# Veason-silverbullet/NNR

Measured on AMD Instinct MI355X. Metric: training impressions/sec on MIND-200k (CNE+SUE, bs=64), higher is better.
Workload: dtype f32

## Files before the change

nnr_amd/csrc/gemm.hip:

```cpp
#include "common.h"
#include <stdlib.h>
#include <type_traits>

namespace {

template <int BK>
__device__ __forceinline__ int swz(int r16) {
  return BK == 16 ? ((4 - (r16 >> 2)) & 3) : BK == 32 ? ((r16 >> 1) & 7) : (r16 & 15);
}

template <int TM, int TN>
__device__ __forceinline__ void gemm_epilogue(const nnr_gemm_args& g, f32x4 (&acc)[TM][TN], float* lds, float* __restrict__ C, int m0,
                                              int n0, int M, int N, int z) {
  constexpr int BN = 16 * TN, E_LD = BN + 4;
  const int tid = threadIdx.x, lane = tid & 63, w = tid >> 6;
  const int r = lane & 15, kk = lane >> 4;
  const uint32_t dthr = g.drop_thresh;
  const float dscale = g.drop_scale;
  const bool use_atomic = !g.slab_mode && (g.atomic || g.split_k > 1 || g.k_chunk > 0);
  float* aux = g.aux_out;
  const float* res = g.resid;
  const float* mulp = g.mul;
  if (g.batch > 1 && g.split_k <= 1 && g.k_chunk <= 0) {
    if (aux) aux += (long)z * g.stride_aux;
// ... 783 lines not shown
  if (nv == TN) run(std::true_type{});
  else run(std::false_type{});
  __syncthreads();
  gemm_epilogue<TM, TN>(g, acc, lds, C, m0, n0, M, N, z);
}

constexpr int kNtRagged = 1;

template <int TM, int TN, int NS, int OCC>
int launch_pipe2(const nnr_gemm_args& g0, hipStream_t s) {
  constexpr int BM = 64 * TM, BN = 16 * TN;
  nnr_gemm_args g = g0;
  g.sched = kNtRagged;
  const int nbm = (g.M + BM - 1) / BM, nbn = (g.N + BN - 1) / BN;
  dim3 grid(nbm * nbn, 1, g.batch > 1 ? g.batch : 1), block(256);
  hipLaunchKernelGGL((gemm_nt_pipe2_kernel<TM, TN, NS, OCC>), grid, block, 0, s, g);
  NNR_CHECK_LAUNCH();
  return NNR_OK;
}

template <int TM, int TN, int BK, int NS, int OCC, int PRIO = 0>
int launch_pipe(const nnr_gemm_args& g0, hipStream_t s) {
  constexpr int BM = 64 * TM, BN = 16 * TN;
  nnr_gemm_args g = g0;
  g.sched = kNtRagged;
  const int nbm = (g.M + BM - 1) / BM, nbn = (g.N + BN - 1) / BN;
  dim3 grid(nbm * nbn, 1, g.batch > 1 ? g.batch : 1), block(256);
  hipLaunchKernelGGL((gemm_nt_pipe_kernel<TM, TN, BK, NS, OCC, PRIO>), grid, block, 0, s, g);
  NNR_CHECK_LAUNCH();
  return NNR_OK;
}

static bool pipe_ok(const nnr_gemm_args& g) {
  auto al = [](const void* p) { return ((uintptr_t)p & 15) == 0; };
  return !g.trans_a && !g.trans_b && !g.b_idx && g.split_k <= 1 && g.k_chunk <= 0 && !g.rowdot_w && !g.colsum_out &&
         (g.drop_target == 0 || g.drop_target == 3 || g.drop_target == 4) && (g.K & 3) == 0 && (g.lda & 3) == 0 && (g.ldb & 3) == 0 &&
         al(g.A) && al(g.B) && (g.batch <= 1 || (((g.strideA | g.strideB) & 3) == 0)) && (g.dyn_dim == 0 || g.dyn_dim == 1);
}

typedef __bf16 bf16x8_t __attribute__((ext_vector_type(8)));
__device__ __forceinline__ void split3_bf16(float x, __bf16& h1, __bf16& h2, __bf16& h3) {
  const unsigned u = __builtin_bit_cast(unsigned, x), mag = u & 0x7fffffffu;
  const bool big = mag >= 0x7f7f8000u, nonfinite = mag >= 0x7f800000u;
  h1 = (__bf16)x;
  if (big) h1 = __builtin_bit_cast(__bf16, (unsigned short)((u >> 16) | (mag > 0x7f800000u ? 0x40u : 0u)));
  const float r1 = nonfinite ? 0.f : x - (float)h1;
  h2 = (__bf16)r1;
  const float r2 = r1 - (float)h2;
  h3 = (__bf16)r2;
}
__global__ void split_bf16x3_kernel(const float* __restrict__ w, int rows, int cols, int ld, int ldo, __bf16* __restrict__ out, long img_stride) {
  const long total = (long)rows * ldo;
  for (long i = blockIdx.x * (long)blockDim.x + threadIdx.x; i < total; i += (long)gridDim.x * blockDim.x) {
    const int r = (int)(i / ldo), c = (int)(i - (long)r * ldo);
    __bf16 a, b, d;
    split3_bf16(c < cols ? w[(long)r * ld + c] : 0.f, a, b, d);
    out[i] = a; out[img_stride + i] = b; out[2 * img_stride + i] = d;
  }
}
__device__ __forceinline__ int bx3_swzA(int r) { return ((r >> 1) & 1) | (((r >> 3) & 1) << 2); }
__device__ __forceinline__ int bx3_swzB(int r) { return (r >> 1) & 3; }

typedef unsigned u32x4_t __attribute__((ext_vector_type(4)));
__device__ __forceinline__ unsigned hi16_pair(float odd, float even) {
  return __builtin_amdgcn_perm(__float_as_uint(odd), __float_as_uint(even), 0x07060302u);
}
__device__ __forceinline__ void split3_trunc8(const f32x4& x0, const f32x4& x1, bf16x8_t& a1, bf16x8_t& a2, bf16x8_t& a3) {
  const float xs[8] = {x0[0], x0[1], x0[2], x0[3], x1[0], x1[1], x1[2], x1[3]};
  unsigned w1[4], w2[4], w3[4];
#pragma unroll
  for (int p = 0; p < 4; ++p) {
    const float xe = xs[2 * p], xo = xs[2 * p + 1];
    const unsigned h1 = hi16_pair(xo, xe);
    const float re = xe - __uint_as_float(h1 << 16), ro = xo - __uint_as_float(h1 & 0xffff0000u);
    const unsigned h2 = hi16_pair(ro, re);
    const float se = re - __uint_as_float(h2 << 16), so = ro - __uint_as_float(h2 & 0xffff0000u);
    w1[p] = h1; w2[p] = h2; w3[p] = hi16_pair(so, se);
  }
  a1 = __builtin_bit_cast(bf16x8_t, u32x4_t{w1[0], w1[1], w1[2], w1[3]});
  a2 = __builtin_bit_cast(bf16x8_t, u32x4_t{w2[0], w2[1], w2[2], w2[3]});
  a3 = __builtin_bit_cast(bf16x8_t, u32x4_t{w3[0], w3[1], w3[2], w3[3]});
}

template <int TM, int TN, int NS>
__global__ __launch_bounds__(256, (NS * (64 * TM * 128 + 3 * 16 * TN * 64) > 80 * 1024 ? 1 : 2)) void gemm_nt_bx3_kernel(nnr_gemm_args g) {
  constexpr int BM = 64 * TM, BN = 16 * TN, BK = 32;
  constexpr int A_BYTES = BM * BK * 4, B_IMG_BYTES = BN * BK * 2, STAGE_BYTES = A_BYTES + 3 * B_IMG_BYTES;
  constexpr int NIA = A_BYTES / 1024, NIB1 = B_IMG_BYTES / 1024;
  static_assert(A_BYTES % 1024 == 0 && B_IMG_BYTES % 1024 == 0 && NIA % 4 == 0, "tile shape");
  constexpr int E_LD = BN + 4;
  constexpr int LDS_BYTES = NS * STAGE_BYTES > 64 * E_LD * 4 ? NS * STAGE_BYTES : 64 * E_LD * 4;
  __shared__ __attribute__((aligned(1024))) unsigned char lds_raw[LDS_BYTES];
  const int tid = threadIdx.x, lane = tid & 63, w = __builtin_amdgcn_readfirstlane(tid >> 6), r = lane & 15, q = lane >> 4;
  int M = g.M;
  if (g.dyn_dim == 1) M = min(M, *g.dyn_dev);
  const int N = g.N, K = g.K;
  const int nbm = (M + BM - 1) / BM, nbn = (N + BN - 1) / BN, nblk = nbm * nbn;
  if ((int)blockIdx.x >= nblk) return;
  int v;
  {
    const int b = blockIdx.x, qq = nblk >> 3, rem = nblk & 7, x = b & 7, slot = b >> 3;
    v = x * qq + min(x, rem) + slot;
  }
  const int bm = v / nbn, bn = v - bm * nbn, m0 = bm * BM, n0 = bn * BN;
  const int S = (K + BK - 1) / BK;
  const unsigned lds_base = (unsigned)(uintptr_t)lds_raw;
  const float* zero = nnr_zero_page;
  asm volatile("" : "+s"(zero));
  constexpr int NA = NIA / 4, NBW = (3 * NIB1 + 3) / 4;
  static_assert(NA <= 8 && NBW <= 8, "tile shape");
  unsigned voffA[8], voffB[8];
  int akc[NA], bkc[NBW];
#pragma unroll
  for (int i = 0; i < 8; ++i) voffA[i] = voffB[i] = 0;
#pragma unroll
  for (int i = 0; i < NA; ++i) {
    const int row = (w + 4 * i) * 8 + lane / 8, c = (lane % 8) ^ bx3_swzA(row & 15);
    akc[i] = 4 * c;
    voffA[i] = (unsigned)(((long)min(row, M - 1 - m0) * g.lda + 4 * c) * 4);
  }
#pragma unroll
  for (int j = 0; j < NBW; ++j) {
    const int idx = min(w + 4 * j, 3 * NIB1 - 1);
    const int img = idx / NIB1, jj = idx - img * NIB1, row = jj * 16 + lane / 4, c = (lane % 4) ^ bx3_swzB(row & 15);
    bkc[j] = 8 * c;
    voffB[j] = (unsigned)(((long)img * g.b3_stride + (long)min(row, N - 1 - n0) * g.ldb3 + 8 * c) * 2);
  }
  const float* Abase = g.A + (long)m0 * g.lda;
  const char* Bbase = reinterpret_cast<const char*>(reinterpret_cast<const __bf16*>(g.B3) + (long)n0 * g.ldb3);
  const bool nb_hi = ((3 * NIB1) % 4 == 0) || (w < (3 * NIB1) % 4);
  const bool ktail = (K % BK) != 0;
  auto issue = [&](int s) __attribute__((always_inline)) {
    const int k0 = s * BK;
    const unsigned sb = lds_base + (unsigned)((s % NS) * STAGE_BYTES) + (unsigned)(w * 1024);
    if (!(ktail && s == S - 1)) {
      lds_dma16_block<NA>(Abase + k0, sb, voffA);
      const float* bb = reinterpret_cast<const float*>(Bbase + 2L * k0);
      if (nb_hi) lds_dma16_block<NBW>(bb, sb + A_BYTES, voffB);
      else if constexpr (NBW > 1) lds_dma16_block<NBW - 1>(bb, sb + A_BYTES, voffB);
      return;
    }
#pragma unroll
    for (int i = 0; i < NA; ++i)
      lds_dma16((k0 + akc[i] < K) ? reinterpret_cast<const float*>(reinterpret_cast<const char*>(Abase + k0) + voffA[i]) : zero, sb + (unsigned)(i * 4096));
#pragma unroll
    for (int j = 0; j < NBW; ++j)
      if (j < NBW - 1 || nb_hi)
        lds_dma16((k0 + bkc[j] < K) ? reinterpret_cast<const float*>(Bbase + 2L * k0 + voffB[j]) : zero, sb + A_BYTES + (unsigned)(j * 4096));
  };
  f32x4 acc_hi[TM][TN], acc_lo[TM][TN];
#pragma unroll
  for (int m = 0; m < TM; ++m)
#pragma unroll
    for (int n = 0; n < TN; ++n) acc_hi[m][n] = acc_lo[m][n] = f32x4{0.f, 0.f, 0.f, 0.f};
#pragma unroll
  for (int s = 0; s < NS - 1; ++s)
    if (s < S) issue(s);
  for (int s = 0; s < S; ++s) {
    if (nb_hi) wait_stages<NA + NBW, NS - 2>(S - 1 - s);
    else wait_stages<NA + NBW - 1, NS - 2>(S - 1 - s);
    __builtin_amdgcn_s_barrier();
    if (s + NS - 1 < S) issue(s + NS - 1);
    const unsigned char* st = lds_raw + (s % NS) * STAGE_BYTES;
    const float* As = reinterpret_cast<const float*>(st);
    const __bf16* Bi = reinterpret_cast<const __bf16*>(st + A_BYTES);
    bf16x8_t bf[3][TN];
#pragma unroll
    for (int img = 0; img < 3; ++img)
#pragma unroll
      for (int n = 0; n < TN; ++n)
        bf[img][n] = *reinterpret_cast<const bf16x8_t*>(Bi + img * (BN * BK) + (n * 16 + r) * BK + ((q ^ bx3_swzB(r)) * 8));
#pragma unroll
    for (int m = 0; m < TM; ++m) {
      const float* arow = As + ((w * TM + m) * 16 + r) * BK;
      const f32x4 x0 = *reinterpret_cast<const f32x4*>(arow + 4 * ((2 * q) ^ bx3_swzA(r)));
      const f32x4 x1 = *reinterpret_cast<const f32x4*>(arow + 4 * ((2 * q + 1) ^ bx3_swzA(r)));
      bf16x8_t a1, a2, a3;
      split3_trunc8(x0, x1, a1, a2, a3);
#pragma unroll
      for (int n = 0; n < TN; ++n) {
        acc_hi[m][n] = __builtin_amdgcn_mfma_f32_16x16x32_bf16(a1, bf[0][n], acc_hi[m][n], 0, 0, 0);
        acc_lo[m][n] = __builtin_amdgcn_mfma_f32_16x16x32_bf16(a3, bf[0][n], acc_lo[m][n], 0, 0, 0);
        acc_lo[m][n] = __builtin_amdgcn_mfma_f32_16x16x32_bf16(a1, bf[2][n], acc_lo[m][n], 0, 0, 0);
        acc_lo[m][n] = __builtin_amdgcn_mfma_f32_16x16x32_bf16(a2, bf[1][n], acc_lo[m][n], 0, 0, 0);
        acc_lo[m][n] = __builtin_amdgcn_mfma_f32_16x16x32_bf16(a2, bf[0][n], acc_lo[m][n], 0, 0, 0);
        acc_lo[m][n] = __builtin_amdgcn_mfma_f32_16x16x32_bf16(a1, bf[1][n], acc_lo[m][n], 0, 0, 0);
      }
    }
  }
#pragma unroll
  for (int m = 0; m < TM; ++m)
#pragma unroll
    for (int n = 0; n < TN; ++n) acc_hi[m][n] += acc_lo[m][n];
  __syncthreads();
  gemm_epilogue<TM, TN>(g, acc_hi, reinterpret_cast<float*>(lds_raw), g.C, m0, n0, M, N, 0);
}

static bool bx3_ok(const nnr_gemm_args& g) {
  auto al = [](const void* p) { return ((uintptr_t)p & 15) == 0; };
  return pipe_ok(g) && !g.a_idx && g.batch <= 1 && g.B3 && al(g.B3) && (g.ldb3 & 7) == 0 && g.ldb3 >= g.K && ((g.b3_stride * 2) & 15) == 0;
}
template <int TM, int TN, int NS>
int launch_bx3(const nnr_gemm_args& g, hipStream_t s) {
  constexpr int BM = 64 * TM, BN = 16 * TN;
  const int nbm = (g.M + BM - 1) / BM, nbn = (g.N + BN - 1) / BN;
  hipLaunchKernelGGL((gemm_nt_bx3_kernel<TM, TN, NS>), dim3(nbm * nbn), dim3(256), 0, s, g);
  NNR_CHECK_LAUNCH();
  return NNR_OK;
}

__device__ __forceinline__ int tn_eff_slices(int split_k, int sched, int K, int nblk, int slots) {
  const int deal_mode = sched & 3;
  const int want_wg = ((sched >> 2) & 63) ? ((sched >> 2) & 63) * 64 : 512;
  const int slice_stages = (sched >> 8) ? (sched >> 8) : 96;
  const int ktiles = (K + 15) / 16;
  const int want = (want_wg + nblk - 1) / nblk;
  int eff = max(1, min(min(split_k, max(want, ktiles / slice_stages)), max(1, ktiles / 12)));
  if (deal_mode != 2) {
    const int W = eff * nblk, wv = W / slots;
    const int target = W < slots ? slots : (((W - wv * slots) * 2 < slots) ? wv * slots : (wv + 1) * slots);
    eff = max(1, min(target / nblk, min(split_k, max(1, ktiles / 12))));
  }
  return eff;
}

template <int TM, int TN, int NS, int OCC, int PRIO = 0>
__global__ __launch_bounds__(256, OCC) void gemm_tn_pipe_kernel(nnr_gemm_args g) {
  if (PRIO == 1) set_prio_dyn((blockIdx.x + gridDim.x * blockIdx.z) >> 8);
  constexpr int BK = 16, BM = 64 * TM, BN = 16 * TN;
  constexpr int PA = BM, PB = BN <= 64 ? 64 : (BN <= 128 ? 128 : 256);
  constexpr int RA = 256 / PA, RB = 256 / PB;
  constexpr int NIA = BK / RA, NIB = BK / RB, NI = NIA + NIB;
  constexpr int NPW = (NI + 3) / 4;
  constexpr int STAGE = BK * (PA + PB);
  constexpr int E_LD = BN + 4;
  constexpr int LDS_FLOATS = (NS * STAGE > 64 * E_LD) ? NS * STAGE : 64 * E_LD;
  static_assert(BN <= 256 && NI % 4 == 0, "tile shape");
  __shared__ __attribute__((aligned(1024))) float lds[LDS_FLOATS];

  const int tid = threadIdx.x, lane = tid & 63, w = __builtin_amdgcn_readfirstlane(tid >> 6);
  const int r = lane & 15, kk = lane >> 4;
  const int M = g.M, N = g.N;
  int K = g.K;
  if (g.dyn_dim == 2) K = min(K, *g.dyn_dev);
  const int nbm = (M + BM - 1) / BM, nbn = (N + BN - 1) / BN;
  const int nblk = nbm * nbn;
  int v, z = 0;
  int kbeg = 0, kend = K;
  if (g.split_k > 1) {
    const int deal_mode = g.sched & 3;
    const int ktiles = (K + BK - 1) / BK;
    const int eff = tn_eff_slices(g.split_k, g.sched, K, nblk, OCC * 256);
    if (deal_mode) {
      const int W = eff * nblk, per = (W + 7) >> 3;
      const int L = blockIdx.x, x = L & 7, slot = L >> 3;
      const int lin = x * per + slot;
      if (slot >= per || lin >= W) return;
      z = lin / nblk;
      v = lin - z * nblk;
    } else {
      z = blockIdx.x / nblk;
      v = blockIdx.x - z * nblk;
      if (z >= eff) return;
    }
    const int per_k = (ktiles + eff - 1) / eff;
    kbeg = z * per_k * BK;
    kend = min(K, kbeg + per_k * BK);
    if (kbeg >= kend) return;
  } else {
    const int b = blockIdx.x, q = nblk >> 3, rem = nblk & 7, x = b & 7, slot = b >> 3;
    v = x * q + min(x, rem) + slot;
  }
  const int bm = v / nbn, bn = v - bm * nbn;
  const int m0 = bm * BM, n0 = bn * BN;
  const float* __restrict__ A = g.A;
  const float* __restrict__ B = g.B;
  const int* __restrict__ bidx = g.b_idx;
  const float* zero = nnr_zero_page;
  asm volatile("" : "+s"(zero));

  long coloff[NPW];
  int krow[NPW];
#pragma unroll
  for (int i = 0; i < NPW; ++i) {
    const int q = w + 4 * i;
    if (q < NIA) {
      const int kl = q * RA + lane / (PA / 4), p4 = lane % (PA / 4);
      const int col = (4 * p4) ^ (16 * ((kl >> 2) & 1));
      krow[i] = kl;
// ... 486 lines not shown
}

int launch_skinny(const nnr_gemm_args& g, hipStream_t s) {
  const int tiles = ((g.M + 15) / 16) * ((g.N + 79) / 80) * (g.batch > 1 ? g.batch : 1);
  dim3 grid(((g.M + 15) / 16) * ((g.N + 79) / 80), 1, g.batch > 1 ? g.batch : 1);
  const bool w8 = tiles <= 640 && g.K >= 384;
#define NNR_SKINNY(TBV, NWV) hipLaunchKernelGGL((skinny_gemm_kernel<TBV, NWV>), grid, dim3(64 * NWV), 0, s, g)
  if (g.trans_b) { if (w8) NNR_SKINNY(true, 8); else NNR_SKINNY(true, 4); }
  else { if (w8) NNR_SKINNY(false, 8); else NNR_SKINNY(false, 4); }
#undef NNR_SKINNY
  NNR_CHECK_LAUNCH();
  return NNR_OK;
}

__global__ __launch_bounds__(256) void splitk_reduce_kernel(const float* __restrict__ slab, const float* __restrict__ cs_slab, float* __restrict__ C,
                                                            int ldc, float* __restrict__ colsum_out, int M, int N, int K, const int* __restrict__ dyn_dev,
                                                            int split_k, int sched, int nblk, int slots, int bk, int kind) {
  if (dyn_dev) K = min(K, *dyn_dev);
  int live;
  const int ktiles = (K + bk - 1) / bk;
  if (ktiles <= 0) {
    live = 0;
  } else if (kind == 1) {
    const int eff = tn_eff_slices(split_k, sched, K, nblk, slots);
    const int per_k = (ktiles + eff - 1) / eff;
    live = min(eff, (ktiles + per_k - 1) / per_k);
  } else {
    const int per = (ktiles + split_k - 1) / split_k;
    live = per > 0 ? min(split_k, (ktiles + per - 1) / per) : 0;
  }
  const long MN = (long)M * N, MN4 = MN >> 2;
  const long stride = (long)gridDim.x * blockDim.x;
  for (long i = blockIdx.x * (long)blockDim.x + threadIdx.x; i < MN4; i += stride) {
    f32x4 t = {0.f, 0.f, 0.f, 0.f};
    int z = 0;
    for (; z + 4 <= live; z += 4) {
      f32x4 v[4];
#pragma unroll
      for (int u = 0; u < 4; ++u) v[u] = reinterpret_cast<const f32x4*>(slab + (long)(z + u) * MN)[i];
#pragma unroll
      for (int u = 0; u < 4; ++u) t += v[u];
    }
    for (; z < live; ++z) t += reinterpret_cast<const f32x4*>(slab + (long)z * MN)[i];
    const long e = i << 2;
    const int m = (int)(e / N), n = (int)(e - (long)m * N);
    float* cp = C + (long)m * ldc + n;
#pragma unroll
    for (int q = 0; q < 4; ++q) atomicAdd(cp + q, t[q]);
  }
  if (colsum_out != nullptr && cs_slab != nullptr) {
    for (long m = blockIdx.x * (long)blockDim.x + threadIdx.x; m < M; m += stride) {
      float t = 0.f;
      for (int z = 0; z < live; ++z) t += cs_slab[(long)z * M + m];
      atomicAdd(&colsum_out[m], t);
    }
  }
}

}

static bool tile_shape(int tile, int* bm, int* bn, int* bk, int* occ, int* kind) {
  struct T { int tile, bm, bn, bk, occ, kind; };
  static const T tab[] = {{2, 64, 80, 16, 1, 0}, {3, 128, 208, 16, 1, 0}, {4, 128, 80, 16, 1, 0}, {5, 128, 80, 32, 1, 0}, {6, 64, 80, 64, 1, 0},
                          {20, 128, 80, 16, 3, 1}, {26, 128, 80, 16, 3, 1}, {27, 128, 208, 16, 2, 1}, {30, 128, 160, 16, 2, 1}, {32, 64, 208, 16, 2, 1}};
  for (const T& t : tab)
    if (t.tile == tile) { *bm = t.bm; *bn = t.bn; *bk = t.bk; *occ = t.occ; *kind = t.kind; return true; }
  return false;
}

static int dispatch_tile(int tile, const nnr_gemm_args& g, hipStream_t stream) {
  switch (tile) {
    case 2: return launch_cfg<1, 5, 16>(g, stream);
    case 3: return launch_cfg<2, 13, 16>(g, stream);
    case 4: return launch_cfg<2, 5, 16>(g, stream);
    case 5: return launch_cfg<2, 5, 32>(g, stream);
    case 6: return launch_cfg<1, 5, 64>(g, stream);
    case 9:  if (!pipe_ok(g) || g.a_idx) return NNR_ERR_ARG; return launch_pipe2<2, 5, 3, 2>(g, stream);
    case 15: if (!pipe_ok(g)) return NNR_ERR_ARG; return launch_pipe<2, 5, 16, 3, 4>(g, stream);
    case 16: if (!pipe_ok(g)) return NNR_ERR_ARG; return launch_pipe<2, 5, 16, 2, 5>(g, stream);
    case 20: if (!tn_pipe_ok(g)) return NNR_ERR_ARG; return launch_tn_pipe<2, 5, 3, 3>(g, stream);
    case 26: if (!tn_pipe_ok(g) || g.b_idx) return NNR_ERR_ARG; return launch_tn_pipe2<2, 5, 3, 3>(g, stream);
    case 27: if (!tn_pipe_ok(g)) return NNR_ERR_ARG; return launch_tn_pipe2<2, 13, 3, 2>(g, stream);
    case 30: if (!tn_pipe_ok(g)) return NNR_ERR_ARG; return launch_tn_pipe2<2, 10, 3, 2>(g, stream);
    case 50: if (!bx3_ok(g)) return NNR_ERR_ARG; return launch_bx3<2, 5, 2>(g, stream);
    case 51: if (!bx3_ok(g)) return NNR_ERR_ARG; return launch_bx3<1, 5, 2>(g, stream);
    case 32: if (!tn_pipe_ok(g)) return NNR_ERR_ARG; return launch_tn_pipe2<1, 13, 3, 2>(g, stream);
    case 7:
      if (g.pre_add || g.gate_bwd) return NNR_ERR_ARG;
      if (g.trans_a || g.a_idx || g.b_idx || g.c_idx || g.dyn_dev || g.split_k > 1 || g.k_chunk > 0 || g.rowdot_w || g.colsum_out || g.atomic ||
          (g.drop_target != 0 && g.drop_target != 3)) return NNR_ERR_ARG;
      return launch_skinny(g, stream);
    default: return NNR_ERR_ARG;
  }
}

extern "C" int nnr_split_bf16x3(const float* w, int rows, int cols, int ld, int ldo, void* out3, long img_stride, hipStream_t stream) {
  if (!w || !out3 || rows <= 0 || cols <= 0 || ld < cols || ldo < cols || (ldo & 7) || img_stride < (long)rows * ldo) return NNR_ERR_ARG;
  const long total = (long)rows * ldo;
  const int blocks = (int)((total + 255) / 256 > 1024 ? 1024 : (total + 255) / 256);
  hipLaunchKernelGGL(split_bf16x3_kernel, dim3(blocks), dim3(256), 0, stream, w, rows, cols, ld, ldo, reinterpret_cast<__bf16*>(out3), img_stride);
  NNR_CHECK_LAUNCH();
  return NNR_OK;
}

extern "C" int nnr_gemm_f32(const nnr_gemm_args* a, hipStream_t stream) {
  if (!a || !a->A || !a->B) return NNR_ERR_ARG;
  if (!a->C && !a->rowdot_out && !a->aux_out) return NNR_ERR_ARG;
  if (a->M <= 0 || a->N <= 0 || a->K <= 0) return NNR_OK;
  nnr_gemm_args g = *a;
  g.drop_thresh = nnr_drop_thresh(g.drop_target ? g.drop_p : 0.f);
  g.drop_scale = (g.drop_target && g.drop_p > 0.f) ? 1.f / (1.f - g.drop_p) : 1.f;
  if (g.drop_thresh == 0u) g.drop_target = 0;
  if (g.k_chunk > 0) { if ((g.k_chunk & 31) || g.batch > 1) return NNR_ERR_ARG; g.split_k = 2; }
  if (g.split_k > 1 && (g.bias || g.rowvec || g.act || g.aux_out || g.mul || g.resid || g.batch > 1 || g.rowdot_w))
    return NNR_ERR_ARG;
  if ((g.a_idx && g.trans_a) || (g.b_idx && !g.trans_b)) return NNR_ERR_ARG;
  if (g.colsum_out && !g.trans_a) return NNR_ERR_ARG;
  if ((g.dyn_dim != 0) != (g.dyn_dev != nullptr)) return NNR_ERR_ARG;
  {
    auto ok = [](const void* p, int ld) { return p == nullptr || ((((uintptr_t)p) & 15) == 0 && (ld & 3) == 0); };
    const bool strides = g.batch <= 1 || (((g.strideC | g.stride_aux | g.stride_res) & 3) == 0);
    g.vec_epi = (!g.c_idx && !g.atomic && g.split_k <= 1 && !g.rowdot_w && (g.N & 3) == 0 && ok(g.C, g.ldc) && ok(g.bias, 0) &&
                 ok(g.rowvec, g.ldrv) && ok(g.aux_out, g.ldaux) && ok(g.mul, g.ldmul) && ok(g.resid, g.ldres) && strides &&
                 (g.drop_target != 3 || (g.drop_cols & 3) == 0)) ? 1 : 0;
  }
  if (g.pre_add || g.gate_bwd) {
    auto al = [](const void* p, int ld) { return p != nullptr && (((uintptr_t)p) & 15) == 0 && (ld & 3) == 0; };
    if (!g.vec_epi || g.split_k > 1 || g.k_chunk > 0 || g.batch > 1 || (g.pre_add && !al(g.pre_add, g.ldpre))) return NNR_ERR_ARG;
    if (g.gate_bwd && (!g.C || !g.aux_out || !g.mul || !g.resid || g.bias || g.rowvec || g.act || g.drop_target || g.accumulate || g.rowdot_w)) return NNR_ERR_ARG;
  }
  float* slab_C = nullptr;
  float* slab_cs = nullptr;
  int slab_ldc = 0;
  if (g.slab != nullptr) {
    if (!(g.trans_a && g.trans_b) || g.split_k <= 1 || g.k_chunk > 0 || g.c_idx || (g.N & 3) || (((uintptr_t)g.slab) & 15) || !g.C || g.accumulate == 2 ||
        g.slab_floats < (long)g.split_k * ((long)g.M * g.N + g.M))
      return NNR_ERR_ARG;
    slab_C = g.C; slab_ldc = g.ldc; slab_cs = g.colsum_out;
    g.C = g.slab; g.ldc = g.N; g.atomic = 0; g.accumulate = 0; g.slab_mode = 1; g.vec_epi = 1;
    if (g.colsum_out) g.colsum_out = g.slab + (long)g.split_k * g.M * g.N;
  } else {
    g.slab_mode = 0;
  }
  int tile = g.tile;
  if (tile == 0) {
    const long wg128 = (long)((g.M + 127) / 128) * ((g.N + 79) / 80) * (g.k_chunk > 0 ? (g.K + g.k_chunk - 1) / g.k_chunk : (g.split_k > 1 ? g.split_k : (g.batch > 1 ? g.batch : 1)));
    const long wg64 = (long)((g.M + 63) / 64) * ((g.N + 79) / 80) * (g.split_k > 1 ? g.split_k : (g.batch > 1 ? g.batch : 1));
    const bool plain = !g.trans_a && !g.a_idx && !g.b_idx && !g.c_idx && !g.dyn_dev && g.split_k <= 1 && g.k_chunk <= 0 && !g.rowdot_w &&
                       !g.colsum_out && !g.atomic && (g.drop_target == 0 || g.drop_target == 3) && !g.pre_add && !g.gate_bwd;
    if (g.rowdot_w) tile = 3;
    else if (plain && wg64 <= 512 && g.K >= 64) tile = 7;
    else if (pipe_ok(g) && !g.a_idx && g.K >= 800 && wg64 > 512) {
      tile = 9;
    }
    else if (pipe_ok(g) && (g.dyn_dev || wg128 >= 640)) tile = 15;
    else if (pipe_ok(g) && wg64 > 512 && g.K >= 128) tile = 16;
    else if (wg64 <= 512 && !g.dyn_dev && g.k_chunk <= 0 && g.K >= 128 && !g.trans_a) tile = 6;
    else if (g.M <= 512 || (wg128 < 640 && !g.dyn_dev)) tile = 2;
    else if (g.trans_a) tile = 2;
    else if (!g.trans_a && !g.trans_b) tile = 5;
    else tile = 4;
  }
  const int rc = dispatch_tile(tile, g, stream);
  if (rc != NNR_OK || !g.slab_mode) return rc;
  int bm, bn, bk, occ, kind;
  if (!tile_shape(tile, &bm, &bn, &bk, &occ, &kind)) return NNR_ERR_ARG;
  const int nblk = ((g.M + bm - 1) / bm) * ((g.N + bn - 1) / bn);
  const long mn4 = ((long)g.M * g.N) >> 2;
// ... 7 lines not shown
```

nnr_amd/ops.py:

```python
import ctypes as C
import math
import os
import weakref

import torch

from . import _lib as L
from . import profile as _prof
from . import tape as _tape

ACT_NONE, ACT_RELU, ACT_TANH, ACT_SIGMOID = 0, 1, 2, 3
K_CHUNK = 1024


class _NoSpan:
    def __enter__(self):
        return self

    def __exit__(self, *a):
        return False


_NOSPAN = _NoSpan()

# ... 257 lines not shown
        launch()
        _refreshed([(e, stamp) for e, _, stamp in jobs], _s())
    for e, _, _ in jobs:
        e.served = False


def wt(w):
    rows, cols = w.shape
    e = _derived('wt', w, (rows, cols), lambda: torch.empty((cols, rows), device=w.device, dtype=torch.float32), isinstance(w, torch.nn.Parameter))
    _serve(e, (w,), lambda: transpose2d(w, e.out, rows, cols))
    return e.out


def wt_prefetch(dev):
    if torch.cuda.is_current_stream_capturing():
        return
    jobs = _stale('wt')
    if not jobs:
        return
    descs = tuple((w.data_ptr(), e.out.data_ptr(), w.shape[0], w.shape[1]) for e, w, _ in jobs)
    if _WT_DESCS[0] != descs:
        arr = (L.TransposeDesc * len(descs))()
        for d, (src, out, rows, cols) in zip(arr, descs):
            d.inp, d.out, d.rows, d.cols = src, out, rows, cols
        _WT_DESCS[:] = [descs, torch.frombuffer(bytearray(bytes(arr)), dtype=torch.uint8).to(dev)]
    table = _WT_DESCS[1]
    tape_keep(table, *[e.out for e, _, _ in jobs])
    _on_leaf(dev, jobs, lambda: L.check(L.lib().nnr_transpose_batch(_p(table), len(descs), _s()), 'nnr_transpose_batch'))


def _pack_entry(lstm, p, H, E):
    return _derived('lstm', lstm, (H, E), lambda: LstmPacked(p, H, E, fill=False), False)


def lstm_pack(lstm, H, E):
    p = lstm.param_list()
    e = _pack_entry(lstm, p, H, E)
    _serve(e, p, lambda: e.out.pack(p))
    return e.out


def lstm_prefetch(dev, lstms, H, E):
    jobs = []
    for lstm in lstms:
        p = lstm.param_list()
        e = _pack_entry(lstm, p, H, E)
        stamp = _stamp(p)
        if e.stamp != stamp:
            jobs.append((e, p, stamp))

    def launch():
        for e, p, _ in jobs:
            tape_keep(*e.bufs)
            e.out.pack(p)
    if jobs:
        _on_leaf(dev, jobs, launch)


def tn_tile(M, N, K, gather=False):
    if K >= 2048 and M >= 512 and N >= 512 and not gather and not ((M & 3) or (N & 3)):
        return 26, 128, 80, 2048
    if K < 8192 or (M & 3) or (N & 3) or (M >= 512 and N >= 512):
        return 0, 64, 80, 2048
    if not gather and M >= 1024 and 160 < N <= 320:
        return 30, 128, 160, 2048
    if N <= 208 or (N > 320 and N <= 416):
        if gather or M % 128 != 0:
            return 32, 64, 208, 640
        return 27, 128, 208, 640
    if gather:
        return 20, 128, 80, 2048
    return 26, 128, 80, 2048


def split_for(m, n, k, tile_m=64, tile_n=80, target_blocks=2048, kmin=256):
    tiles = max(1, ((m + tile_m - 1) // tile_m) * ((n + tile_n - 1) // tile_n))
    if k <= 640:
        return 1
    return int(max(1, min((k + kmin - 1) // kmin, (target_blocks + tiles - 1) // tiles)))


BX3 = [os.environ.get('NNR_BX3', '1') == '1']
_BX3_MIN_ROWS = 2048
_BX3_TILE = 50
_BX3_CLASSES = {'dx', 'sue', 'proj', 'gate'}


def bx3_class(N, K):
    if K >= 1024:
        return 'dx'
    if K >= 800:
        return 'sue'
    if N >= 1024:
        return 'proj'
    return 'gate'


BX3_SEEN = {}


def _split_bf16x3(B, N, K, ldb, img):
    ldo = img.shape[2]
    L.check(L.lib().nnr_split_bf16x3(_p(B), N, K, ldb, ldo, _p(img), N * ldo, _s()), 'nnr_split_bf16x3')


def bx3_prefetch(dev):
    if not BX3[0] or torch.cuda.is_current_stream_capturing():
        return
    jobs = _stale('bx3')

    def launch():
        for e, B, _ in jobs:
            tape_keep(e.out, B)
            _split_bf16x3(B, *e.spec, e.out)
    if jobs:
        _on_leaf(dev, jobs, launch)


def bx3_images(B, N, K, ldb):
    ldo = (K + 7) // 8 * 8
    owner = _OWNED.get(id(B))
    e = _derived('bx3', B, (N, K, ldb), lambda: torch.empty((3, N, ldo), device=B.device, dtype=torch.int16),
                 isinstance(B, torch.nn.Parameter) or (owner is not None and owner.prefetch))
    _serve(e, (B,), lambda: _split_bf16x3(B, N, K, ldb, e.out))
    return e.out, N * ldo, ldo


def _bx3_wanted(A, B, M, N, K, lda, ldb, trans_a, trans_b, a_idx, b_idx, c_idx, split_k, k_chunk, rowdot_w, colsum_out, atomic, batch, dyn_dim, drop):
    return (not trans_a and not trans_b and a_idx is None and b_idx is None and split_k <= 1 and k_chunk <= 0 and rowdot_w is None
            and colsum_out is None and batch <= 1 and dyn_dim in (0, 1) and M >= _BX3_MIN_ROWS and K >= 64 and N * K <= (1 << 22)
            and (K | lda | ldb) & 3 == 0 and (A.data_ptr() | B.data_ptr()) & 15 == 0 and (drop is None or drop[0] in (3, 4) or drop[1] <= 0.0))


def gemm(A, B, C_=None, *, M, N, K, lda, ldb, ldc=0, trans_a=False, trans_b=False, dyn=None, dyn_dim=0, a_idx=None, b_idx=None,
         drop=None, alpha=1.0, bias=None, rowvec=None, ldrv=0, rowvec_map=None, act=0, aux_out=None, ldaux=0, mul=None, ldmul=0,
         resid=None, ldres=0, accumulate=False, atomic=False, c_idx=None, split_k=1, rowdot_w=None, rowdot_out=None, batch=1,
         strideA=0, strideB=0, strideC=0, stride_aux=0, stride_res=0, tile=0, colsum_out=None, k_chunk=0, flop_scale=1.0, slab=None,
         pre_add=None, ldpre=0, gate_bwd=False, b3=None):
    g = L.GemmArgs()
    g.A, g.B = A.data_ptr(), B.data_ptr()
    if C_ is not None:
        g.C = C_.data_ptr()
    g.M, g.N, g.K, g.lda, g.ldb, g.ldc, g.alpha = M, N, K, lda, ldb, ldc, alpha
    if trans_a:
        g.trans_a = 1
    if trans_b:
        g.trans_b = 1
    if dyn is not None:
        g.dyn_dev, g.dyn_dim = dyn.data_ptr(), dyn_dim
    if a_idx is not None:
        g.a_idx = a_idx.data_ptr()
    if b_idx is not None:
        g.b_idx = b_idx.data_ptr()
    if drop is not None and drop[1] > 0.0:
        g.drop_target, g.drop_p, g.drop_seed, g.drop_cols = drop[0], float(drop[1]), int(drop[2]), int(drop[3])
    if bias is not None:
        g.bias = bias.data_ptr()
    if rowvec is not None:
        g.rowvec, g.ldrv, g.rowvec_map = rowvec.data_ptr(), ldrv, _p(rowvec_map)
    if act:
        g.act = act
    if aux_out is not None:
        g.aux_out, g.ldaux = aux_out.data_ptr(), ldaux
    if mul is not None:
        g.mul, g.ldmul = mul.data_ptr(), ldmul
    if resid is not None:
        g.resid, g.ldres = resid.data_ptr(), ldres
    if accumulate:
        g.accumulate = int(accumulate)
    if atomic:
        g.atomic = 1
    if c_idx is not None:
        g.c_idx = c_idx.data_ptr()
    g.split_k, g.batch = int(split_k), batch
    if rowdot_w is not None:
        g.rowdot_w, g.rowdot_out = rowdot_w.data_ptr(), rowdot_out.data_ptr()
    if batch > 1:
        g.strideA, g.strideB, g.strideC, g.stride_aux, g.stride_res = strideA, strideB, strideC, stride_aux, stride_res
    if tile:
        g.tile = tile
    if colsum_out is not None:
        g.colsum_out = colsum_out.data_ptr()
    if k_chunk:
        g.k_chunk = int(k_chunk)
    if pre_add is not None:
        g.pre_add, g.ldpre = pre_add.data_ptr(), ldpre
    if gate_bwd:
        g.gate_bwd = 1
    if b3 is None and BX3[0] and tile in (0, 9, 15, 16) and _bx3_wanted(A, B, M, N, K, lda, ldb, trans_a, trans_b, a_idx, b_idx, c_idx, split_k, k_chunk, rowdot_w,
                                                                    colsum_out, atomic, batch, dyn_dim, drop):
        is_w = is_weight(B)
        key = (M, N, K, 'weight' if is_w else 'other')
        BX3_SEEN[key] = BX3_SEEN.get(key, 0) + 1
        if is_w and bx3_class(N, K) in _BX3_CLASSES:
            b3 = bx3_images(B, N, K, ldb)
            tile = _BX3_TILE
            g.tile = _BX3_TILE
    if b3 is not None:
        g.B3, g.b3_stride, g.ldb3 = b3[0].data_ptr(), b3[1], b3[2]
    if slab is None and TN_SLAB and trans_a and trans_b and split_k > 1 and not k_chunk and c_idx is None and (N & 3) == 0 and C_ is not None:
        slab = _slab_ws(A.device, int(split_k) * (M * N + M))
    if slab is not None:
        g.slab, g.slab_floats = slab.data_ptr(), slab.numel()
    if not (A.is_cuda and B.is_cuda):
        raise L.NnrHipError('nnr_amd ops need device tensors (no CPU fallback on the product path)')
    if not _prof.active():
        L.check(L.lib().nnr_gemm_f32(C.byref(g), _s()), 'nnr_gemm_f32')
        return
    pipe_nt = (not trans_a and not trans_b and b_idx is None and split_k <= 1 and k_chunk <= 0 and rowdot_w is None and colsum_out is None
               and (drop is None or drop[0] in (3, 4) or drop[1] <= 0.0) and (K | lda | ldb) & 3 == 0 and (A.data_ptr() | B.data_ptr()) & 15 == 0)
    wg128 = ((M + 127) // 128) * ((N + 79) // 80) * (split_k if split_k > 1 else max(1, batch)) * (1 if k_chunk <= 0 else max(1, K // k_chunk))
    wg64 = ((M + 63) // 64) * ((N + 79) // 80) * (split_k if split_k > 1 else max(1, batch))
    if tile:
        t = tile
    elif rowdot_w is not None:
        t = 3
    elif (not trans_a and a_idx is None and b_idx is None and c_idx is None and dyn is None and split_k <= 1 and k_chunk <= 0
          and colsum_out is None and not atomic and wg64 <= 512 and K >= 64 and drop is None):
        t = 7
    elif pipe_nt and a_idx is None and K >= 800 and wg64 > 512:
        t = 9
    elif pipe_nt and (dyn is not None or wg128 >= 640):
        t = 15
    elif pipe_nt and wg64 > 512 and K >= 128:
        t = 16
    elif wg64 <= 512 and dyn is None and k_chunk <= 0 and K >= 128:
        t = 6
    elif M <= 512 or (wg128 < 640 and dyn is None) or trans_a:
        t = 2
    else:
        t = 5 if not trans_b else 4
    fam = 'gemm_%s_%s' % ('tn' if trans_a else ('nn' if trans_b else 'nt'),
                          {2: '64x80', 3: '128x208', 4: '128x80', 5: '128x80k32', 6: '64x80k64', 7: '16x80skinny', 9: 'pipe2_128x80', 15: 'pipe128x80', 16: 'pipe128x80s2',
                           20: 'pipe128x80', 26: 'pipe2_128x80', 27: 'pipe2_128x208', 30: 'pipe2_128x160', 32: 'pipe2_64x208', 50: 'bx3_128x80', 51: 'bx3_64x80'}.get(t, 'tile%d' % t))

    def flops(vals=None, M=M, N=N, K=K, dyn=dyn, dyn_dim=dyn_dim, batch=batch):
        m, k = M, K
        if dyn is not None:
            d = int(vals[dyn.data_ptr()]) if vals is not None else int(dyn.item())
            m, k = (min(M, d), K) if dyn_dim == 1 else (M, min(K, d))
        return 2.0 * m * N * k * max(1, batch) * flop_scale
    flops.dyn = [dyn] if dyn is not None else []
    flops.scale = flop_scale

    def op_bytes(vals=None, M=M, N=N, K=K, dyn=dyn, dyn_dim=dyn_dim, batch=batch):
        m, k = M, K
        if dyn is not None:
            d = int(vals[dyn.data_ptr()]) if vals is not None else int(dyn.item())
            m, k = (min(M, d), K) if dyn_dim == 1 else (M, min(K, d))
        outs = (1 if C_ is not None else 0) + (1 if accumulate else 0) + (1 if aux_out is not None else 0) + (1 if mul is not None else 0) + (1 if resid is not None else 0) + (1 if pre_add is not None else 0)
        return 4.0 * max(1, batch) * (m * k + N * k + m * N * outs)
    flops.bytes_fn = op_bytes
    if trans_a and trans_b and split_k > 1:
        flops.tn_dims = (M, N, flop_scale)
    flops.tag = 'M%d N%d K%d%s%s%s' % (M, N, K, ' b%d' % batch if batch > 1 else '', (' sk%d' % split_k if split_k > 1 else '') + (' kc%d' % k_chunk if k_chunk > 0 else ''), ' dyn' if dyn is not None else '')
    with _prof.span(fam, flops):
        L.check(L.lib().nnr_gemm_f32(C.byref(g), _s()), 'nnr_gemm_f32')


def linear_fwd(x, w, bias=None, out=None, act=0, **kw):
    M, K = x.shape
    N = w.shape[0]
    if out is None:
        out = torch.empty((M, N), device=x.device, dtype=torch.float32)
    gemm(x, w, out, M=M, N=N, K=K, lda=x.stride(0), ldb=w.stride(0), ldc=out.stride(0), bias=bias, act=act, **kw)
    return out


def linear_bwd_data(dy, w, out=None, accumulate=False, **kw):
    M, N = dy.shape
    K = w.shape[1]
    if out is None:
        out = torch.empty((M, K), device=dy.device, dtype=torch.float32)
    if M >= 1024 and w.is_contiguous() and (N & 3) == 0:
        gemm(dy, wt(w), out, M=M, N=K, K=N, lda=dy.stride(0), ldb=N, ldc=out.stride(0), accumulate=accumulate, **kw)
    else:
        gemm(dy, w, out, M=M, N=K, K=N, lda=dy.stride(0), ldb=w.stride(0), ldc=out.stride(0), trans_b=True, accumulate=accumulate, **kw)
    return out


def linear_bwd_weight(dy, x, dw, dyn=None, rows=None, db=None, small_lds=False, **kw):
    R = dy.shape[0] if rows is None else rows
    N, K = dw.shape
    t, bm, bn, target = tn_tile(N, K, R)
    if small_lds:
        t, bm, bn, target = 2, 64, 80, 2048
    if t and ((dy.stride(0) | x.stride(0)) & 3 or (dy.data_ptr() | x.data_ptr()) & 15):
        t, bm, bn, target = 0, 64, 80, 2048
    gemm(dy, x, dw, M=N, N=K, K=R, lda=dy.stride(0), ldb=x.stride(0), ldc=dw.stride(0), trans_a=True, trans_b=True,
         atomic=True, dyn=dyn, dyn_dim=2, colsum_out=db, split_k=split_for(N, K, R, bm, bn, target), tile=t, **kw)


def rowdot(x, w, out, dyn=None, rows=None):
    R = x.shape[0] if rows is None else rows
    L.check(L.lib().nnr_rowdot(_p(x), x.stride(0), _p(w), _p(dyn), R, x.shape[1], _p(out), _s()), 'nnr_rowdot')


_SLOT_WS = {}
_SLAB_WS = {}
TN_SLAB = True
def _slab_ws(dev, floats):
    key = torch._C._cuda_getCurrentRawStream(dev.index if dev.index is not None else torch.cuda.current_device())
    ws = _SLAB_WS.get(key)
    if ws is None or ws.numel() < floats:
        ws = torch.empty(max(int(floats), 1 << 22), device=dev, dtype=torch.float32)
        _SLAB_WS[key] = ws
    tape_keep(ws)
    return ws



def _slot_ws(dev, n):
    key = torch._C._cuda_getCurrentRawStream(dev.index if dev.index is not None else torch.cuda.current_device())
    need = L.lib().nnr_slot_workspace_floats(n)
    ws = _SLOT_WS.get(key)
    if ws is None or ws.numel() < need:
        ws = torch.zeros(max(need, 32 * 1024), device=dev, dtype=torch.float32)
# ... 1099 lines not shown
```

nnr_amd/profile.py:

```python
import os

import torch

_on = False
_records = []

KERNEL_OF = {
    'gemm_nt_256x80': 'gemm_kernel<4, 5, false, false, 16>', 'gemm_nn_256x80': 'gemm_kernel<4, 5, false, true, 16>',
    'gemm_tn_256x80': 'gemm_kernel<4, 5, true, true, 16>', 'gemm_nt_64x80': 'gemm_kernel<1, 5, false, false, 16>',
    'gemm_nn_64x80': 'gemm_kernel<1, 5, false, true, 16>', 'gemm_tn_64x80': 'gemm_kernel<1, 5, true, true, 16>',
    'gemm_nt_128x208': 'gemm_kernel<2, 13, false, false, 16>', 'gemm_nt_128x80': 'gemm_kernel<2, 5, false, false, 16>', 'gemm_nt_128x80k32': 'gemm_kernel<2, 5, false, false, 32>',
    'gemm_nt_64x80k64': 'gemm_kernel<1, 5, false, false, 64>', 'gemm_nn_64x80k64': 'gemm_kernel<1, 5, false, true, 64>',
    'gemm_tn_64x80k64': 'gemm_kernel<1, 5, true, true, 64>',
    'gemm_nt_pipe128x80': 'gemm_nt_pipe_kernel<2, 5, 16, 3, 4, 0>', 'gemm_nt_pipe128x80s2': 'gemm_nt_pipe_kernel<2, 5, 16, 2, 5, 0>',
    'gemm_nt_bx3_128x80': 'gemm_nt_bx3_kernel<2, 5, 2>', 'gemm_nt_bx3_64x80': 'gemm_nt_bx3_kernel<1, 5, 2>',
    'gemm_nt_pipe2_128x80': 'gemm_nt_pipe2_kernel<2, 5, 3, 2>', 'gemm_nt_pipe2_128x64': 'gemm_nt_pipe2_kernel<2, 4, 3, 2>',
    'gemm_tn_pipe2_128x80': 'gemm_tn_pipe2_kernel<2, 5, 3, 3>', 'gemm_tn_pipe2_128x208': 'gemm_tn_pipe2_kernel<2, 13, 3, 2>', 'gemm_tn_pipe2_128x160': 'gemm_tn_pipe2_kernel<2, 10, 3, 2>', 'gemm_tn_pipe2_64x208': 'gemm_tn_pipe2_kernel<1, 13, 3, 2>',
    'gemm_tn_pipe128x80': 'gemm_tn_pipe_kernel<2, 5, 3, 3, 0>', 'gemm_tn_pipe128x208': 'gemm_tn_pipe_kernel<2, 13, 3, 2, 0>',
    'gemm_nn_128x80': 'gemm_kernel<2, 5, false, true, 16>', 'gemm_tn_128x80': 'gemm_kernel<2, 5, true, true, 16>', 'lstm_fwd': 'lstm_fwd_pair_kernel<13>', 'lstm_bwd': 'lstm_bwd_pair_kernel<13, true>',
    'gru_fwd': 'gru_fwd_kernel<13>', 'gru_bwd': 'gru_bwd_kernel<13>',
}


_enabled, _every = False, 1
TAPE_HOOK = [None]
TAPE_RECORDS = []


_eager = True


def enable(every=1, eager=True):
    global _on, _enabled, _every, _eager
    _enabled, _every, _eager = True, max(1, int(every)), bool(eager)
    _on = _eager
    _records.clear()
    TAPE_RECORDS.clear()


def begin_step(i):
    global _on
    inst = _enabled and (i % _every == 0)
    _on = inst and _eager
    return inst


def disable():
    global _on, _enabled
    _on = _enabled = False


def active():
    return _on or TAPE_HOOK[0] is not None


class span:

    def __init__(self, family, flops_fn):
        self.family, self.flops_fn = family, flops_fn

    def __enter__(self):
        if TAPE_HOOK[0] is not None:
            TAPE_HOOK[0](self.family, self.flops_fn)
        if _on:
            self.s = torch.cuda.Event(enable_timing=True)
            self.e = torch.cuda.Event(enable_timing=True)
            self.s.record()
        return self

    def __exit__(self, *a):
        if _on:
            self.e.record()
            _records.append((self.family, self.s, self.e, self.flops_fn))
        return False


def by_shape():
    out = {}
    for family, fn, ms in _all_records():
        tag = getattr(fn, 'tag', '')
        d = out.setdefault((family, tag), dict(ms=0.0, flops=0.0, launches=0))
        d['ms'] += ms
        d['flops'] += float(fn())
        d['launches'] += 1
    return out


def _all_records():
    torch.cuda.synchronize()
    for family, s, e, fn in _records:
        yield family, fn, s.elapsed_time(e)
    for family, fn, ms in TAPE_RECORDS:
        yield family, fn, ms


def _bytes_of(fn):
    if hasattr(fn, 'op_bytes'):
        return float(fn.op_bytes)
# ... 249 lines not shown
```

Measured before the change: 6765.

## Split bx3 GEMM staging into separate A and B LDS rings

Refactors the bx3 split-bf16 GEMM so the fp32 A tile and the three bf16 B images use independent LDS ring buffers with their own depths. B for the next step and A further ahead are issued separately, and the wait counts only A DMA groups. A 3-deep-A variant is added, and the default tile switches to a new 2/2 ring configuration. This is meant to reduce LDS footprint and stalls from the combined stage wait, at the risk of subtle ordering errors in the counted wait.

Result: no change. 6723 (median of 2 runs) (-0.6%).

```diff
diff --git a/nnr_amd/csrc/gemm.hip b/nnr_amd/csrc/gemm.hip
--- a/nnr_amd/csrc/gemm.hip
+++ b/nnr_amd/csrc/gemm.hip
@@ -889,14 +889,15 @@
   a3 = __builtin_bit_cast(bf16x8_t, u32x4_t{w3[0], w3[1], w3[2], w3[3]});
 }
 
-template <int TM, int TN, int NS>
-__global__ __launch_bounds__(256, (NS * (64 * TM * 128 + 3 * 16 * TN * 64) > 80 * 1024 ? 1 : 2)) void gemm_nt_bx3_kernel(nnr_gemm_args g) {
+template <int TM, int TN, int NSA, int NSB>
+__device__ __forceinline__ void gemm_nt_bx3_body(const nnr_gemm_args& g) {
   constexpr int BM = 64 * TM, BN = 16 * TN, BK = 32;
-  constexpr int A_BYTES = BM * BK * 4, B_IMG_BYTES = BN * BK * 2, STAGE_BYTES = A_BYTES + 3 * B_IMG_BYTES;
+  constexpr int A_BYTES = BM * BK * 4, B_IMG_BYTES = BN * BK * 2, B_BYTES = 3 * B_IMG_BYTES, RING_BYTES = NSA * A_BYTES + NSB * B_BYTES;
   constexpr int NIA = A_BYTES / 1024, NIB1 = B_IMG_BYTES / 1024;
   static_assert(A_BYTES % 1024 == 0 && B_IMG_BYTES % 1024 == 0 && NIA % 4 == 0, "tile shape");
+  static_assert(NSB == 2 && (NSA == NSB || NSA == NSB + 1), "the issue order and the counted wait below are derived for these rings");
   constexpr int E_LD = BN + 4;
-  constexpr int LDS_BYTES = NS * STAGE_BYTES > 64 * E_LD * 4 ? NS * STAGE_BYTES : 64 * E_LD * 4;
+  constexpr int LDS_BYTES = RING_BYTES > 64 * E_LD * 4 ? RING_BYTES : 64 * E_LD * 4;
   __shared__ __attribute__((aligned(1024))) unsigned char lds_raw[LDS_BYTES];
   const int tid = threadIdx.x, lane = tid & 63, w = __builtin_amdgcn_readfirstlane(tid >> 6), r = lane & 15, q = lane >> 4;
   int M = g.M;
@@ -937,40 +938,43 @@
   const char* Bbase = reinterpret_cast<const char*>(reinterpret_cast<const __bf16*>(g.B3) + (long)n0 * g.ldb3);
   const bool nb_hi = ((3 * NIB1) % 4 == 0) || (w < (3 * NIB1) % 4);
   const bool ktail = (K % BK) != 0;
-  auto issue = [&](int s) __attribute__((always_inline)) {
+  auto issueA = [&](int s) __attribute__((always_inline)) {
     const int k0 = s * BK;
-    const unsigned sb = lds_base + (unsigned)((s % NS) * STAGE_BYTES) + (unsigned)(w * 1024);
-    if (!(ktail && s == S - 1)) {
-      lds_dma16_block<NA>(Abase + k0, sb, voffA);
-      const float* bb = reinterpret_cast<const float*>(Bbase + 2L * k0);
-      if (nb_hi) lds_dma16_block<NBW>(bb, sb + A_BYTES, voffB);
-      else if constexpr (NBW > 1) lds_dma16_block<NBW - 1>(bb, sb + A_BYTES, voffB);
-      return;
-    }
+    const unsigned sb = lds_base + (unsigned)((s % NSA) * A_BYTES) + (unsigned)(w * 1024);
+    if (!(ktail && s == S - 1)) { lds_dma16_block<NA>(Abase + k0, sb, voffA); return; }
 #pragma unroll
     for (int i = 0; i < NA; ++i)
       lds_dma16((k0 + akc[i] < K) ? reinterpret_cast<const float*>(reinterpret_cast<const char*>(Abase + k0) + voffA[i]) : zero, sb + (unsigned)(i * 4096));
+  };
+  auto issueB = [&](int s) __attribute__((always_inline)) {
+    const int k0 = s * BK;
+    const unsigned sb = lds_base + (unsigned)(NSA * A_BYTES + (s % NSB) * B_BYTES) + (unsigned)(w * 1024);
+    if (!(ktail && s == S - 1)) {
+      const float* bb = reinterpret_cast<const float*>(Bbase + 2L * k0);
+      if (nb_hi) lds_dma16_block<NBW>(bb, sb, voffB);
+      else if constexpr (NBW > 1) lds_dma16_block<NBW - 1>(bb, sb, voffB);
+      return;
+    }
 #pragma unroll
     for (int j = 0; j < NBW; ++j)
       if (j < NBW - 1 || nb_hi)
-        lds_dma16((k0 + bkc[j] < K) ? reinterpret_cast<const float*>(Bbase + 2L * k0 + voffB[j]) : zero, sb + A_BYTES + (unsigned)(j * 4096));
+        lds_dma16((k0 + bkc[j] < K) ? reinterpret_cast<const float*>(Bbase + 2L * k0 + voffB[j]) : zero, sb + (unsigned)(j * 4096));
   };
   f32x4 acc_hi[TM][TN], acc_lo[TM][TN];
 #pragma unroll
   for (int m = 0; m < TM; ++m)
 #pragma unroll
     for (int n = 0; n < TN; ++n) acc_hi[m][n] = acc_lo[m][n] = f32x4{0.f, 0.f, 0.f, 0.f};
-#pragma unroll
-  for (int s = 0; s < NS - 1; ++s)
-    if (s < S) issue(s);
+  issueA(0);
+  issueB(0);
+  if constexpr (NSA > NSB) if (1 < S) issueA(1);
   for (int s = 0; s < S; ++s) {
-    if (nb_hi) wait_stages<NA + NBW, NS - 2>(S - 1 - s);
-    else wait_stages<NA + NBW - 1, NS - 2>(S - 1 - s);
+    wait_stages<NA, NSA - 2>(S - 1 - s);
     __builtin_amdgcn_s_barrier();
-    if (s + NS - 1 < S) issue(s + NS - 1);
-    const unsigned char* st = lds_raw + (s % NS) * STAGE_BYTES;
-    const float* As = reinterpret_cast<const float*>(st);
-    const __bf16* Bi = reinterpret_cast<const __bf16*>(st + A_BYTES);
+    if (s + 1 < S) issueB(s + 1);
+    if (s + NSA - 1 < S) issueA(s + NSA - 1);
+    const float* As = reinterpret_cast<const float*>(lds_raw + (s % NSA) * A_BYTES);
+    const __bf16* Bi = reinterpret_cast<const __bf16*>(lds_raw + NSA * A_BYTES + (s % NSB) * B_BYTES);
     bf16x8_t bf[3][TN];
 #pragma unroll
     for (int img = 0; img < 3; ++img)
@@ -1002,16 +1006,22 @@
   __syncthreads();
   gemm_epilogue<TM, TN>(g, acc_hi, reinterpret_cast<float*>(lds_raw), g.C, m0, n0, M, N, 0);
 }
+constexpr int bx3_occ(int TM, int TN, int NSA, int NSB) { return NSA * 64 * TM * 128 + NSB * 3 * 16 * TN * 64 > 80 * 1024 ? 1 : 2; }
+template <int TM, int TN, int NS>
+__global__ __launch_bounds__(256, bx3_occ(TM, TN, NS, NS)) void gemm_nt_bx3_kernel(nnr_gemm_args g) { gemm_nt_bx3_body<TM, TN, NS, NS>(g); }
+template <int TM, int TN, int NSA, int NSB>
+__global__ __launch_bounds__(256, bx3_occ(TM, TN, NSA, NSB)) void gemm_nt_bx3_rings_kernel(nnr_gemm_args g) { gemm_nt_bx3_body<TM, TN, NSA, NSB>(g); }
 
 static bool bx3_ok(const nnr_gemm_args& g) {
   auto al = [](const void* p) { return ((uintptr_t)p & 15) == 0; };
   return pipe_ok(g) && !g.a_idx && g.batch <= 1 && g.B3 && al(g.B3) && (g.ldb3 & 7) == 0 && g.ldb3 >= g.K && ((g.b3_stride * 2) & 15) == 0;
 }
-template <int TM, int TN, int NS>
+template <int TM, int TN, int NSA, int NSB>
 int launch_bx3(const nnr_gemm_args& g, hipStream_t s) {
   constexpr int BM = 64 * TM, BN = 16 * TN;
   const int nbm = (g.M + BM - 1) / BM, nbn = (g.N + BN - 1) / BN;
-  hipLaunchKernelGGL((gemm_nt_bx3_kernel<TM, TN, NS>), dim3(nbm * nbn), dim3(256), 0, s, g);
+  if constexpr (NSA == NSB) hipLaunchKernelGGL((gemm_nt_bx3_kernel<TM, TN, NSB>), dim3(nbm * nbn), dim3(256), 0, s, g);
+  else hipLaunchKernelGGL((gemm_nt_bx3_rings_kernel<TM, TN, NSA, NSB>), dim3(nbm * nbn), dim3(256), 0, s, g);
   NNR_CHECK_LAUNCH();
   return NNR_OK;
 }
@@ -1664,8 +1674,9 @@
     case 26: if (!tn_pipe_ok(g) || g.b_idx) return NNR_ERR_ARG; return launch_tn_pipe2<2, 5, 3, 3>(g, stream);
     case 27: if (!tn_pipe_ok(g)) return NNR_ERR_ARG; return launch_tn_pipe2<2, 13, 3, 2>(g, stream);
     case 30: if (!tn_pipe_ok(g)) return NNR_ERR_ARG; return launch_tn_pipe2<2, 10, 3, 2>(g, stream);
-    case 50: if (!bx3_ok(g)) return NNR_ERR_ARG; return launch_bx3<2, 5, 2>(g, stream);
-    case 51: if (!bx3_ok(g)) return NNR_ERR_ARG; return launch_bx3<1, 5, 2>(g, stream);
+    case 50: if (!bx3_ok(g)) return NNR_ERR_ARG; return launch_bx3<2, 5, 3, 2>(g, stream);
+    case 51: if (!bx3_ok(g)) return NNR_ERR_ARG; return launch_bx3<1, 5, 2, 2>(g, stream);
+    case 52: if (!bx3_ok(g)) return NNR_ERR_ARG; return launch_bx3<2, 5, 2, 2>(g, stream);
     case 32: if (!tn_pipe_ok(g)) return NNR_ERR_ARG; return launch_tn_pipe2<1, 13, 3, 2>(g, stream);
     case 7:
       if (g.pre_add || g.gate_bwd) return NNR_ERR_ARG;
diff --git a/nnr_amd/ops.py b/nnr_amd/ops.py
--- a/nnr_amd/ops.py
+++ b/nnr_amd/ops.py
@@ -363,7 +363,8 @@
 
 BX3 = [os.environ.get('NNR_BX3', '1') == '1']
 _BX3_MIN_ROWS = 2048
-_BX3_TILE = 50
+_BX3_TILE = 52
+_BX3_CLASS_TILE = {}
 _BX3_CLASSES = {'dx', 'sue', 'proj', 'gate'}
 
 
@@ -475,8 +476,8 @@
         BX3_SEEN[key] = BX3_SEEN.get(key, 0) + 1
         if is_w and bx3_class(N, K) in _BX3_CLASSES:
             b3 = bx3_images(B, N, K, ldb)
-            tile = _BX3_TILE
-            g.tile = _BX3_TILE
+            tile = _BX3_CLASS_TILE.get(bx3_class(N, K), _BX3_TILE)
+            g.tile = tile
     if b3 is not None:
         g.B3, g.b3_stride, g.ldb3 = b3[0].data_ptr(), b3[1], b3[2]
     if slab is None and TN_SLAB and trans_a and trans_b and split_k > 1 and not k_chunk and c_idx is None and (N & 3) == 0 and C_ is not None:
@@ -513,7 +514,7 @@
         t = 5 if not trans_b else 4
     fam = 'gemm_%s_%s' % ('tn' if trans_a else ('nn' if trans_b else 'nt'),
                           {2: '64x80', 3: '128x208', 4: '128x80', 5: '128x80k32', 6: '64x80k64', 7: '16x80skinny', 9: 'pipe2_128x80', 15: 'pipe128x80', 16: 'pipe128x80s2',
-                           20: 'pipe128x80', 26: 'pipe2_128x80', 27: 'pipe2_128x208', 30: 'pipe2_128x160', 32: 'pipe2_64x208', 50: 'bx3_128x80', 51: 'bx3_64x80'}.get(t, 'tile%d' % t))
+                           20: 'pipe128x80', 26: 'pipe2_128x80', 27: 'pipe2_128x208', 30: 'pipe2_128x160', 32: 'pipe2_64x208', 50: 'bx3_128x80_a3', 51: 'bx3_64x80', 52: 'bx3_128x80'}.get(t, 'tile%d' % t))
 
     def flops(vals=None, M=M, N=N, K=K, dyn=dyn, dyn_dim=dyn_dim, batch=batch):
         m, k = M, K
diff --git a/nnr_amd/profile.py b/nnr_amd/profile.py
--- a/nnr_amd/profile.py
+++ b/nnr_amd/profile.py
@@ -13,7 +13,7 @@
     'gemm_nt_64x80k64': 'gemm_kernel<1, 5, false, false, 64>', 'gemm_nn_64x80k64': 'gemm_kernel<1, 5, false, true, 64>',
     'gemm_tn_64x80k64': 'gemm_kernel<1, 5, true, true, 64>',
     'gemm_nt_pipe128x80': 'gemm_nt_pipe_kernel<2, 5, 16, 3, 4, 0>', 'gemm_nt_pipe128x80s2': 'gemm_nt_pipe_kernel<2, 5, 16, 2, 5, 0>',
-    'gemm_nt_bx3_128x80': 'gemm_nt_bx3_kernel<2, 5, 2>', 'gemm_nt_bx3_64x80': 'gemm_nt_bx3_kernel<1, 5, 2>',
+    'gemm_nt_bx3_128x80': 'gemm_nt_bx3_kernel<2, 5, 2>', 'gemm_nt_bx3_64x80': 'gemm_nt_bx3_kernel<1, 5, 2>', 'gemm_nt_bx3_128x80_a3': 'gemm_nt_bx3_rings_kernel<2, 5, 3, 2>',
     'gemm_nt_pipe2_128x80': 'gemm_nt_pipe2_kernel<2, 5, 3, 2>', 'gemm_nt_pipe2_128x64': 'gemm_nt_pipe2_kernel<2, 4, 3, 2>',
     'gemm_tn_pipe2_128x80': 'gemm_tn_pipe2_kernel<2, 5, 3, 3>', 'gemm_tn_pipe2_128x208': 'gemm_tn_pipe2_kernel<2, 13, 3, 2>', 'gemm_tn_pipe2_128x160': 'gemm_tn_pipe2_kernel<2, 10, 3, 2>', 'gemm_tn_pipe2_64x208': 'gemm_tn_pipe2_kernel<1, 13, 3, 2>',
     'gemm_tn_pipe128x80': 'gemm_tn_pipe_kernel<2, 5, 3, 3, 0>', 'gemm_tn_pipe128x208': 'gemm_tn_pipe_kernel<2, 13, 3, 2, 0>',
```
